# 51616/split-vae

Hardware: AMD Instinct MI355X
Metric: images/sec training step, SPLIT-VAE CelebA-64 bs512 (higher is better)
Workload: dtype f32 operands, f32 accumulate (exact-fp32 MFMA v_mfma_f32_16x16x4_f32): the reference's precision (vae/model.py:12); 1 GPU; SPLIT-VAE CelebA-64 64x64 beta=120 patch_size=8 latents=128+128 lr=1e-4, full train step (scramble+fwd+ELBO+bwd+Adam), per-GPU batch 512; global_batch=512, per_gpu_batch=512, parallelism=dp1, reconstructions=not stored (dead after the fused loss)

## Files before the change

### split_vae_amd/csrc/kernels.h

```cpp
#pragma once
#include <hip/hip_runtime.h>
#include <stdint.h>

#define SV_MAX_TAPS 81

struct TapGemmArgs {
  const void* A;
  const void* Wt;
  const float* bias;
  void* out;
  const void* mask;
  int M;
  int lOY, lOX;
  int OY, OX;
  int IH, IW, lda;
  int cl2;
  int P;
  int Ktot;
  int S, SX;
  int N;
  int OHF, OWF, OS, ooy, oox, ldo;
  int act, out_f32, splitk, ntaps;
  int ups;
  int d2s;
  int d2s_y;
  int clampin;
  int s2d3;
  const float* nll_img; void* nll_grad; float* nll_part; int nll_ch; float nll_gscale;
  int nll_noout;
  const float* fix;
  const float* fix2; int fix_nc, fix_pad;
  int cls_n;
  int accum;
  int adj;
  int8_t dy[SV_MAX_TAPS];
  int8_t dx[SV_MAX_TAPS];
};
int svk_tap_gemm(const TapGemmArgs& a, int dtype, int cfg, hipStream_t st);
#define SV_TAP_MAX_MULTI 4
struct TapGemmMulti {
  TapGemmArgs a[SV_TAP_MAX_MULTI];
  int zbase[SV_TAP_MAX_MULTI];
  int n;
};
int svk_tap_gemm_multi(const TapGemmArgs* a, int n, int dtype, int cfg, hipStream_t st);

struct TileConvArgs {
  const void* A; const void* Wt; const float* bias; void* out; const void* mask;
  int B, IH, IW, lda;
  int cl2, P, Ktot, S, SX;
  int lTW, lTH, lNB;
  int OY, OX, tilesX, tilesY, ntiles;
  int TIW, TIH, y_lo, x_lo;
  int PS;
  int plane_bytes;
  int nph, lnph;
  int xcd_chunk;
  int off_bytes, in_bytes;
  int buf_bytes;
  int wslots;
  int N, OHF, OWF, OS, ooy, oox, ldo, act, out_f32, ntaps;
  int dbg;
  int ups;
  int d2s;
  int cls_n;
  int d2s_y, clampin;
  int s2d3;
  int dma;
  const float* fix;
  const float* fix2; int fix_nc, fix_pad;
  const float* nll_img; void* nll_grad; float* nll_part; int nll_ch; float nll_gscale; int nll_noout;
  int8_t dy[SV_MAX_TAPS];
  int8_t dx[SV_MAX_TAPS];
};
#define SV_MAX_MULTI 8
#define SV_SHARED_STREAMS 3
hipStream_t sv_shared_stream(int k);
struct TileConvMulti { TileConvArgs a[SV_MAX_MULTI]; };
bool svk_tile_conv_plan(const TapGemmArgs& t, int dtype, int B, TileConvArgs* a, int* cfg_out);
int svk_tile_conv_multi(const TileConvArgs* a, int n, int dtype, int cfg, hipStream_t st);
int svk_conv_dispatch_multi(const TapGemmArgs* t, int n, int dtype, int tap_cfg, hipStream_t st);
int svk_tile_conv(const TileConvArgs& a, int dtype, int cfg, hipStream_t st);
int svk_row_conv_try(const TapGemmArgs* t, int n, int dtype, hipStream_t st);
bool svk_row_conv_supported(const TapGemmArgs* t, int n, int dtype);
int svk_conv_dispatch(const TapGemmArgs& t, int dtype, int tap_cfg, hipStream_t st);

struct WgradArgs {
  const void* A;
  const void* dY;
  float* dW;
  float* dbias;
  int M, lOY, lOX, OY, OX, IH, IW, lda, S, SX;
  int fold_kw, fold_c;
  int ldy, ycols;
  int cl2;
  int Cin_pad, Cin_real, N, Nrows;
  int ntaps, msplit;
  int ups;
  int clampin;
  int dy_s2d;
  int dy_os, dy_oy, dy_ox;
  int assign;
  int s2d3;
  float* ws;
  int64_t ws_bytes;
  hipEvent_t ev_mid[2];
  struct WgradReduceDesc* defer; int* n_defer;
  int8_t dy[SV_MAX_TAPS];
  int8_t dx[SV_MAX_TAPS];
};
int svk_wgrad(const WgradArgs& a, int dtype, int cfg, hipStream_t st);
#define SV_WGRAD_IM2COL_MAX_MULTI 4
struct WgradMulti {
  WgradArgs a[SV_WGRAD_IM2COL_MAX_MULTI];
  int zbase[SV_WGRAD_IM2COL_MAX_MULTI];
  int plain[SV_WGRAD_IM2COL_MAX_MULTI];
  int n;
};
int svk_wgrad_multi(const WgradArgs* a, int n, int dtype, int cfg, hipStream_t st);

struct WgradTileArgs {
  const void* A; const void* dY; float* dW; float* dbias;
  float* slab; float* ws; int64_t ws_bytes;
  float* bslab;
  struct WgradReduceDesc* defer; int* n_defer;
  int B, IH, IW, lda, cl2, S, SX, fold_kw, fold_c;
  int layer_id;
  int contig;
  int pairx;
  int lTW, lTH, lNB, OY, OX, tilesX, tilesY, ntiles;
  int TIW, TIH, y_lo, x_lo, PS;
  int ldy, YS, lycp;
  int in_bytes, dy_bytes;
  int dbg;
  int ups;
  int clampin, dy_s2d, assign;
  int dy_os, dy_oy, dy_ox;
  int s2d3;
// ... 131 lines not shown
```

### split_vae_amd/csrc/tile_conv.hip

```cpp
#include "common.hip.h"
#include "kernels.h"
#include "tile_stage.hip.h"
#include "dlogistic.hip.h"
#include <stdio.h>
#include <stdlib.h>
#include <string.h>

#ifndef SV_TC_PPS16
#define SV_TC_PPS16 16
#endif
#ifndef SV_TC_PPS32
#define SV_TC_PPS32 8
#endif
#ifndef SV_TC_PPS64
#define SV_TC_PPS64 8
#endif
#ifndef SV_TC_EPI_BATCH
#define SV_TC_EPI_BATCH 8
#endif
static __host__ __device__ constexpr int tile_pps(int BN, int YR = 0) {
  return YR ? (BN == 16 || YR == 5 ? YR * 4 : 8) : BN == 16 ? SV_TC_PPS16 : BN == 32 ? SV_TC_PPS32 : BN == 64 ? SV_TC_PPS64 : 8;
}

template <int PPS>
__device__ __forceinline__ int wpiece(int q, int n) {
  if constexpr (PPS % 8 == 0) return q ^ (n & 7);
  else return (q & ~7) == (PPS & ~7) ? (q & ~3) | ((q & 3) ^ (n & 3)) : q ^ (n & 7);
}

template <typename T> struct MmaOpT;
template <> struct MmaOpT<bf16_t> {
  static __device__ __forceinline__ void run(const uint4& a, const uint4& b, f32x4& c) {
    c = __builtin_amdgcn_mfma_f32_16x16x32_bf16(__builtin_bit_cast(bf16x8, a), __builtin_bit_cast(bf16x8, b), c, 0, 0, 0);
  }
};
template <> struct MmaOpT<float> {
  static __device__ __forceinline__ void run(const uint4& a, const uint4& b, f32x4& c) {
    const float4 af = __builtin_bit_cast(float4, a), bf = __builtin_bit_cast(float4, b);
    c = __builtin_amdgcn_mfma_f32_16x16x4f32(af.x, bf.x, c, 0, 0, 0);
    c = __builtin_amdgcn_mfma_f32_16x16x4f32(af.y, bf.y, c, 0, 0, 0);
    c = __builtin_amdgcn_mfma_f32_16x16x4f32(af.z, bf.z, c, 0, 0, 0);
    c = __builtin_amdgcn_mfma_f32_16x16x4f32(af.w, bf.w, c, 0, 0, 0);
  }
};

static constexpr int tile_min_waves(int BN, int NW, int YR, bool WR = false) { return (YR || WR) && NW == 4 ? (BN == 64 ? 3 : 4) : 1; }
template <typename T, int BN, int MF, int NW, int YR, bool WR, bool FX = false>
__global__ __launch_bounds__(64 * NW, tile_min_waves(BN, NW, YR, WR)) void tile_conv_kernel(const TileConvMulti mg) {
  const TileConvArgs& g = mg.a[blockIdx.z];
  if (SV_DBG(g.dbg) & 32) return;
  constexpr int NT = 64 * NW, WM = 16 * MF, BM = NW * WM, NF = BN / 16;
  constexpr int PPS = tile_pps(BN, YR), RB = PPS * 16;
  constexpr int RPP = NT / PPS;
  constexpr int BRN = (BN + RPP - 1) / RPP;
  constexpr int EPP = ElemTraits<T>::EPP;
  extern __shared__ __attribute__((aligned(16))) char smem[];
  char* sB = smem;
  int* sOff = (int*)(smem + g.wslots * BN * RB);
  char* sIn = smem + g.wslots * BN * RB + g.off_bytes;

  const int tid = threadIdx.x, lane = tid & 63, wave = tid >> 6;
  int t = blockIdx.x;
  if (g.xcd_chunk) {
    const int remapped = (t & 7) * g.xcd_chunk + (t >> 3);
    t = remapped < g.ntiles && (g.ntiles & 7) == 0 ? remapped : t;
  }
  const int tx0 = (t % g.tilesX) << g.lTW; t /= g.tilesX;
  const int ty0 = (t % g.tilesY) << g.lTH; t /= g.tilesY;
  const int b0 = t << g.lNB;
  const int n0 = blockIdx.y * BN;
  const int TW = 1 << g.lTW, TH = 1 << g.lTH, NB = 1 << g.lNB;
  const int cpp = 1 << g.cl2;

  const T* __restrict__ Wb = (const T*)g.Wt;
  const int nph = g.nph, lcH = g.cl2 - g.lnph;
  const int gP = g.P >> g.lnph, gKtot = g.Ktot, gdbg = SV_DBG(g.dbg);
  const int pp = tid % PPS, r0 = tid / PPS;
  int ph = 0;
  uint4 rbA[BRN];
  auto load_b = [&](int ks, uint4 (&rb)[BRN]) {
    const int pl = ks * PPS + pp;
    const bool pv = pl < gP;
    const int p = ((pl >> lcH) << g.cl2) + (ph << lcH) + (pl & ((1 << lcH) - 1));
#pragma unroll
    for (int i = 0; i < BRN; ++i) {
      const int n = r0 + RPP * i;
      rb[i] = (pv && n < BN && r0 < RPP) ? *(const uint4*)(Wb + (int64_t)(n0 + n) * gKtot + (int64_t)p * EPP) : make_uint4(0, 0, 0, 0);
    }
  };
  auto write_b = [&](int slot, const uint4 (&rb)[BRN]) {
#pragma unroll
    for (int i = 0; i < BRN; ++i) {
      const int n = r0 + RPP * i;
      if (n < BN && r0 < RPP) *(uint4*)(sB + slot * (BN * RB) + n * RB + (wpiece<PPS>(pp, n) << 4)) = rb[i];
    }
  };
  const int nk = (gdbg & 2) ? 0 : (gP + PPS - 1) / PPS;
  constexpr int WRMAX = 6;
  constexpr bool wres = WR && YR == 0;
  uint4 rbw[wres ? WRMAX - 1 : 1][BRN];
  load_b(0, rbA);
  if constexpr (wres) {
#pragma unroll
    for (int ks = 1; ks < WRMAX; ++ks) load_b(ks, rbw[ks - 1]);
  }

  const int nkp = (gP + PPS - 1) / PPS * PPS;
  for (int p = tid; p < nkp; p += NT) {
    int off = 0;
    if (p < gP) {
      const int tap = p >> lcH, c = p & ((1 << lcH) - 1);
      const int tp = ((int)g.dy[tap] - g.y_lo) * g.TIW + ((int)g.dx[tap] - g.x_lo);
      off = g.plane_bytes ? tp * 32 + (c >> 1) * g.plane_bytes + (c & 1) * 16 : tp * g.PS + c * 16;
    }
    sOff[p] = off;
  }
  auto stage = [&](int phase) {
    if (SV_DBG(g.dbg) & 1) return;
    const TileStageGeom sg = {g.B, g.IH, g.IW, g.lda, lcH, g.TIW, g.TIH, g.PS, NB, g.plane_bytes};
    const int iy_base = ty0 * g.S + g.y_lo, ix_base = tx0 * g.SX + g.x_lo;
    const T* Ap = (const T*)g.A + ((phase << lcH) * EPP);
    if constexpr (sizeof(T) == 4) {
      if (g.s2d3) { stage_tile_s2d3<NT>((const float*)g.A, sg, b0, iy_base, ix_base, sIn, tid); return; }
    }
    if (g.ups) stage_tile_upsampled<T, NT>(Ap, sg, b0, iy_base, ix_base, sIn, tid);
    else if (sizeof(T) == 4 && g.dma) {
      const int wv = __builtin_amdgcn_readfirstlane(wave);
      if (g.clampin) stage_tile_plain_dma<T, NW, true>(Ap, sg, b0, iy_base, ix_base, sIn, lane, wv);
      else stage_tile_plain_dma<T, NW, false>(Ap, sg, b0, iy_base, ix_base, sIn, lane, wv);
    }
    else if (g.clampin) stage_tile_plain<T, NT, true>(Ap, sg, b0, iy_base, ix_base, sIn, tid);
    else stage_tile_plain<T, NT>(Ap, sg, b0, iy_base, ix_base, sIn, tid);
  };
  stage(0);
  const int lr = lane & 15, lg = lane >> 4;
  int lbase[MF];
#pragma unroll
  for (int i = 0; i < MF; ++i) {
    const int r = wave * WM + i * 16 + lr;
    const int tx = r & (TW - 1), ty = (r >> g.lTW) & (TH - 1), bl = r >> (g.lTW + g.lTH);
    lbase[i] = ((bl * g.TIH + ty * g.S) * g.TIW + tx * g.SX) * g.PS;
  }

  f32x4 acc[MF][NF];
#pragma unroll
  for (int i = 0; i < MF; ++i)
#pragma unroll
    for (int j = 0; j < NF; ++j) acc[i][j] = (f32x4){0.f, 0.f, 0.f, 0.f};

  auto compute = [&](int ks, int slot) {
    const char* cB = sB + slot * (BN * RB);
#pragma unroll
    for (int kk = 0; kk < PPS / 4; ++kk) {
      const int off = sOff[ks * PPS + kk * 4 + lg];
      uint4 af[MF], bfr[NF];
#pragma unroll
      for (int i = 0; i < MF; ++i) af[i] = *(const uint4*)(sIn + lbase[i] + off);
#pragma unroll
      for (int j = 0; j < NF; ++j) {
        const int n = j * 16 + lr;
        bfr[j] = *(const uint4*)(cB + n * RB + (wpiece<PPS>(kk * 4 + lg, n) << 4));
      }
#pragma unroll
      for (int i = 0; i < MF; ++i)
#pragma unroll
        for (int j = 0; j < NF; ++j) MmaOpT<T>::run(bfr[j], af[i], acc[i][j]);
    }
  };
  constexpr int SPG = YR ? YR * 4 / PPS : 1, TPS = PPS / 4;
  const int rowpitch = g.TIW * g.PS;
  for (ph = 0; ph < nph; ++ph) {
    if (ph) {
      load_b(0, rbA);
      stage(ph);
    }
    write_b(0, rbA);
    if constexpr (wres) {
#pragma unroll
      for (int ks = 1; ks < WRMAX; ++ks)
        if (ks < nk) write_b(ks, rbw[ks - 1]);
    }
    __syncthreads();
    if constexpr (YR > 0) {
      for (int gq = 0; gq * SPG < nk; ++gq) {
        uint4 aw[MF + YR - 1];
        const char* wp = sIn + lbase[0] + sOff[gq * (YR * 4) + lg];
#pragma unroll
        for (int iy = 0; iy < MF + YR - 1; ++iy) aw[iy] = *(const uint4*)(wp + iy * rowpitch);
#pragma unroll
        for (int sg = 0; sg < SPG; ++sg) {
          const int ks = gq * SPG + sg;
          const bool more = ks + 1 < nk;
          if (more) load_b(ks + 1, rbA);
          const char* cB = sB + (ks & 1) * (BN * RB);
#pragma unroll
          for (int kk = 0; kk < TPS; ++kk) {
            uint4 bfr[NF];
#pragma unroll
            for (int j = 0; j < NF; ++j) {
              const int n = j * 16 + lr;
              bfr[j] = *(const uint4*)(cB + n * RB + (wpiece<PPS>(kk * 4 + lg, n) << 4));
            }
#pragma unroll
            for (int i = 0; i < MF; ++i)
#pragma unroll
              for (int j = 0; j < NF; ++j) MmaOpT<T>::run(bfr[j], aw[i + sg * TPS + kk], acc[i][j]);
          }
          if (more) write_b((ks & 1) ^ 1, rbA);
          __syncthreads();
        }
      }
    } else if constexpr (wres) {
      for (int ks = 0; ks < nk; ++ks) compute(ks, ks);
      __syncthreads();
    } else
    for (int ks = 0; ks < nk; ++ks) {
      const bool more = ks + 1 < nk && !(gdbg & 8);
      if (more) load_b(ks + 1, rbA);
      compute(ks, ks & 1);
      if (more) write_b((ks & 1) ^ 1, rbA);
      if (!(gdbg & 16)) __syncthreads();
    }
    if (nk == 0) __syncthreads();
  }
// ... 277 lines not shown
  return true;
}
static bool tile_conv_plan_impl(const TapGemmArgs& t, int dtype, int B, TileConvArgs* a, int* cfg_out, bool narrow, int64_t* lds_out) {
  if (t.splitk != 1 || t.accum) return false;
  if (t.lOY < 0 || t.lOX < 0 || t.S > 2) return false;
  const int OY = 1 << t.lOY, OX = 1 << t.lOX;
  if (t.ups && t.S != 1) return false;
  if (t.d2s && ((t.N != 16 && !(t.N == 32 && t.d2s_y)) || !t.out_f32)) return false;
  if (t.d2s_y && (!t.d2s || t.N != 32 || ((2 * t.d2s * 4) & 7))) return false;
  if (t.clampin && (t.ups || t.S != 1)) return false;
  if (t.s2d3 && (dtype != SV_F32 || t.S != 1 || t.SX != 1 || t.ups || t.clampin || t.cl2 != 2)) return false;
  if (t.fix_nc && !t.d2s_y && (dtype != SV_F32 || !t.fix || !t.fix2 || (t.N & 15) || t.out_f32)) return false;
  if (t.nll_part && (!t.d2s_y || t.d2s != 6 || OY * OX < 256 || !t.nll_img || !t.nll_grad)) return false;
  if (t.cls_n && (t.OS != 2 || t.N != 4 * t.cls_n || (t.cls_n & 7) || t.out_f32 || t.bias)) return false;
  if (OY * OX < 16) return false;
  if (!t.d2s && !t.cls_n) {
    const int oe = t.out_f32 ? 4 : (dtype == SV_BF16 ? 2 : 4);
    const int nst = (t.N & 7) ? (t.ldo < ((t.N + 7) & ~7) ? t.ldo : ((t.N + 7) & ~7)) : t.N;
    if ((nst * oe) & 7) return false;
  }
  const int esz = dtype == SV_BF16 ? 2 : 4, epp = 16 / esz;
  const int cin = (1 << t.cl2) * epp;
  int BN, cfgN;
  static const int small_wgs = SV_TUNE_INT("SV_TC_SMALL_WGS", 200);
  const int64_t wgs128 = (((int64_t)B * OY * OX + 127) / 128) * (t.N / 128);
  static const bool small_f32 = SV_TUNE_INT("SV_TC_SMALL_F32", 1) != 0;
  const bool small = t.N % 128 == 0 && (wgs128 < small_wgs || narrow) && (dtype == SV_BF16 || small_f32) && !t.cls_n;
  static const int tiny_wgs = SV_TUNE_INT("SV_TC_TINY_WGS", 100);
  const bool tiny = small && wgs128 < tiny_wgs;
  static const int small64_wgs = SV_TUNE_INT("SV_TC_SMALL64_WGS", 300);
  const int64_t wgs64 = (((int64_t)B * OY * OX + 127) / 128) * (t.N / 64);
  static const int small64_s = SV_TUNE_INT("SV_TC_SMALL64_S", 1);
  const bool tiny64 = dtype == SV_F32 && t.N % 64 == 0 && t.N % 128 != 0 && wgs64 < small64_wgs && !t.cls_n && !t.d2s && t.OS == 1 && (!small64_s || t.S == small64_s);
  if (t.N % 128 == 0 && !small) { BN = 128; cfgN = 0; }
  else if (t.N % 64 == 0 && !tiny && !tiny64) { BN = 64; cfgN = 1; }
  else if (t.N % 32 == 0) { BN = 32; cfgN = 2; }
  else if (t.N <= 16) { BN = 16; cfgN = 3; }
  else return false;
  int y_lo = 127, y_hi = -127, x_lo = 127, x_hi = -127;
  for (int i = 0; i < t.ntaps; ++i) {
    y_lo = t.dy[i] < y_lo ? t.dy[i] : y_lo; y_hi = t.dy[i] > y_hi ? t.dy[i] : y_hi;
    x_lo = t.dx[i] < x_lo ? t.dx[i] : x_lo; x_hi = t.dx[i] > x_hi ? t.dx[i] : x_hi;
  }
  static const bool s2pad = !SV_TUNE_FLAG("SV_TC_NO_S2PAD"), p64 = SV_TUNE_FLAG("SV_TC_PAD64");
  const int pb = cin * esz;
  static const bool planar_on = !SV_TUNE_FLAG("SV_TC_NO_PLANAR");
  auto layout = [&](int bytes, bool* planar_out) {
    const bool pl = planar_on && t.SX == 1 && t.S == 1 && bytes >= 64;
    *planar_out = pl;
    return pl ? 32 : bytes + (t.SX == 1 ? ((bytes >= 128 || (bytes == 64 && p64)) ? 32 : 0) : ((bytes % 32 == 0 && s2pad) ? 16 : 0));
  };
  const int lTW = OX >= 16 ? 4 : t.lOX;
  const int off_bytes = (((t.P + 31) / 32 * 32) * 4 + 15) / 16 * 16;
  static const char* mf2 = SV_TUNE_STR("SV_TC_MF2", nullptr);
  for (int MF = 4; MF >= 2; MF -= 2) {
    static const bool big128 = SV_TUNE_FLAG("SV_TC_BN128_MF4");
    if (MF == 4 && BN == 128 && !(big128 && dtype == SV_BF16)) continue;
    if (MF == 4 && mf2 && strchr(mf2, BN == 16 ? 'a' : BN == 32 ? 'b' : 'c')) continue;
    if (MF == 4 && small) continue;
    if (MF == 4 && BN == 32 && OY * OX <= 256 && t.OS == 2 && !t.d2s_y) continue;
    const int BM = 64 * MF;
    int lTH = 0;
    while ((1 << (lTW + lTH)) < BM && (1 << lTH) < OY) ++lTH;
    int lNB = 0;
    while ((1 << (lTW + lTH + lNB)) < BM) ++lNB;
    const int TW = 1 << lTW, TH = 1 << lTH, NB = 1 << lNB;
    if (t.nll_part && (BM != 256 || NB != 1)) return false;
    const int TIW = (TW - 1) * t.SX + (x_hi - x_lo) + 1, TIH = (TH - 1) * t.S + (y_hi - y_lo) + 1;
    int yr = 0;
    static const char* yr_off = SV_TUNE_STR("SV_TC_NO_YR", "a");
    if (dtype == SV_BF16 && MF == 4 && t.S == 1 && lTW == 4 && TH >= MF && cin >= 32 && BN <= 64 &&
        !(yr_off && (yr_off[0] == '1' || strchr(yr_off, BN == 16 ? 'a' : BN == 32 ? 'b' : 'c')))) {
      int kh = 1;
      while (kh < t.ntaps && t.dx[kh] == t.dx[0]) ++kh;
      bool ok = (kh == 4 || kh == 6) && t.ntaps % kh == 0;
      for (int i = 0; i < t.ntaps && ok; ++i)
        ok = t.dx[i] == t.dx[i / kh * kh] && t.dy[i] == t.dy[0] + i % kh && t.dy[0] == y_lo;
      if (ok) yr = kh;
    }
    static const int nph_max = SV_TUNE_INT("SV_TC_NPH", 4);
    const int64_t wgs = (int64_t)(OX / TW) * (OY / TH) * ((B + NB - 1) / NB) * ((t.N + BN - 1) / BN);
    static const int small32_wgs = SV_TUNE_INT("SV_TC_SMALL32_WGS", 300);
    if (MF == 4 && BN == 32 && dtype == SV_F32 && !t.nll_part && wgs < small32_wgs) continue;
    int lnph = 0, PS = 0, plane_bytes = 0;
    int64_t in_bytes = 0;
    bool planar = false;
    for (;; ++lnph) {
      if (yr) lnph = t.cl2 - 2;
      const int pbh = pb >> lnph;
      PS = layout(pbh, &planar);
      plane_bytes = planar ? NB * TIH * TIW * 32 : 0;
      in_bytes = planar ? (int64_t)plane_bytes * (pbh / 32) : (int64_t)NB * TIH * TIW * PS;
      static const int ph_kb = SV_TUNE_INT("SV_TC_PH_KB", 53);
      static const bool s2_phases = !SV_TUNE_FLAG("SV_TC_NPH_NO_S2");
      static const int ph_wgs = SV_TUNE_INT("SV_TC_PH_WGS", 256);
      const int64_t tot = in_bytes + 2 * BN * tile_pps(BN) * 16 + off_bytes;
      if (yr || t.s2d3 || !((2 << lnph) <= nph_max && (pbh >> 1) >= 32 && (planar || s2_phases) &&
                            ((wgs >= ph_wgs && tot > ph_kb * 1024) || tot > 150 * 1024))) break;
    }
    static const bool wres_on = !SV_TUNE_FLAG("SV_TC_NO_WRES");
    const int nks = (int)(((t.P >> lnph) + tile_pps(BN) - 1) / tile_pps(BN));
    const int wslots = (wres_on && !yr && dtype == SV_BF16 && BN == 32 && MF == 4 && t.S == 1 && lnph == 0 && nks > 2 && nks <= 6 && nks * BN * tile_pps(BN) * 16 <= 24 * 1024) ? nks : 2;
    const int64_t lds = (int64_t)wslots * BN * tile_pps(BN, yr) * 16 + off_bytes + in_bytes;
    if (lds > 78 * 1024 && MF == 4 && BN >= 64) continue;
    static const bool s2_mf4 = SV_TUNE_FLAG("SV_TC_S2_MF4");
    if (lds > 78 * 1024 && MF == 4 && t.S == 2 && t.fix_nc && !s2_mf4) continue;
    *lds_out = lds;
    if (lds > 150 * 1024) {
      if (MF == 4) continue;
      if (SV_TUNE_FLAG("SV_TC_VERBOSE")) fprintf(stderr, "tile_conv plan: REFUSED (LDS %lld) N=%d cin=%d S=%d ntaps=%d\n", (long long)lds, t.N, cin, t.S, t.ntaps);
      return false;
    }
    memset(a, 0, sizeof(*a));
    a->A = t.A; a->Wt = t.Wt; a->bias = t.bias; a->out = t.out; a->mask = t.mask;
    a->B = B; a->IH = t.IH; a->IW = t.IW; a->lda = t.lda;
    a->cl2 = t.cl2; a->P = t.P; a->Ktot = t.Ktot; a->S = t.S; a->SX = t.SX; a->d2s = t.d2s; a->cls_n = t.cls_n; a->d2s_y = t.d2s_y; a->clampin = t.clampin; a->fix = t.fix;
    a->fix2 = t.fix2; a->fix_nc = t.d2s_y ? 0 : t.fix_nc; a->fix_pad = t.fix_pad; a->s2d3 = t.s2d3;
    a->nll_img = t.nll_img; a->nll_grad = t.nll_grad; a->nll_part = t.nll_part; a->nll_ch = t.nll_ch; a->nll_gscale = t.nll_gscale; a->nll_noout = t.nll_noout;
    a->lTW = lTW; a->lTH = lTH; a->lNB = lNB;
    a->OY = OY; a->OX = OX;
    a->tilesX = OX / TW; a->tilesY = OY / TH;
    a->ntiles = a->tilesX * a->tilesY * ((B + NB - 1) / NB);
    a->TIW = TIW; a->TIH = TIH; a->y_lo = y_lo; a->x_lo = x_lo; a->PS = PS; a->plane_bytes = plane_bytes;
    a->nph = 1 << lnph; a->lnph = lnph; a->wslots = wslots;
    {
      static const bool no_dma = SV_TUNE_FLAG("SV_TC_NO_DMA");
      a->dma = (!no_dma && dtype == SV_F32 && !t.ups && !t.s2d3 && (planar || PS == (pb >> lnph))) ? 1 : 0;
    }
    if (SV_TUNE_FLAG("SV_TC_VERBOSE")) fprintf(stderr, "tile_conv plan: yr=%d wslots=%d N=%d BN=%d MF=%d cin=%d pb=%d planar=%d nph=%d tile=%dx%dx%d PS=%d in_bytes=%lld lds=%lld ntiles=%d S=%d SX=%d\n", yr, wslots, t.N, BN, MF, cin, pb, (int)planar, 1 << lnph, NB, TIH, TIW, PS, (long long)in_bytes, (long long)lds, a->ntiles, t.S, t.SX);
    {
      static const bool xcd = !SV_TUNE_FLAG("SV_TC_NO_XCD");
      a->xcd_chunk = (xcd && a->ntiles >= 64 && (a->ntiles & 7) == 0) ? a->ntiles / 8 : 0;
    }
    a->off_bytes = off_bytes; a->in_bytes = (int)in_bytes;
    a->N = t.N; a->OHF = t.OHF; a->OWF = t.OWF; a->OS = t.OS; a->ooy = t.ooy; a->oox = t.oox; a->ldo = t.ldo;
    a->act = t.act; a->out_f32 = t.out_f32; a->ntaps = t.ntaps; a->ups = t.ups;
    memcpy(a->dy, t.dy, sizeof(a->dy));
    memcpy(a->dx, t.dx, sizeof(a->dx));
    *cfg_out = cfgN * 2 + (MF == 4 ? 0 : 1) + (yr == 4 ? 32 : yr == 6 ? 64 : 0) + (wslots > 2 ? 128 : 0);
    static const char* nw8 = SV_TUNE_STR("SV_TC_NW8", nullptr);
    if (MF == 4 && dtype == SV_BF16 && nw8 && strchr(nw8, BN == 16 ? 'a' : BN == 32 ? 'b' : BN == 64 ? 'c' : 'd')) *cfg_out = 16 + cfgN;
    return true;
  }
  return false;
}

int svk_tile_conv_multi(const TileConvArgs* a, int n, int dtype, int cfg, hipStream_t st) {
  if (n < 1 || n > SV_MAX_MULTI) return SV_E_BADARG;
  if (dtype == SV_BF16) {
    switch (cfg) {
      case 0: return launch_tile<bf16_t, 128, 4>(a, n, st);
      case 1: return launch_tile<bf16_t, 128, 2>(a, n, st);
      case 2: return launch_tile<bf16_t, 64, 4>(a, n, st);
      case 3: return launch_tile<bf16_t, 64, 2>(a, n, st);
      case 4: return launch_tile<bf16_t, 32, 4>(a, n, st);
      case 5: return launch_tile<bf16_t, 32, 2>(a, n, st);
      case 7: return launch_tile<bf16_t, 16, 2>(a, n, st);
      case 6: return launch_tile<bf16_t, 16, 4>(a, n, st);
      case 128 + 4: return launch_tile<bf16_t, 32, 4, 4, 0, true>(a, n, st);
      case 32 + 2: return launch_tile<bf16_t, 64, 4, 4, 4>(a, n, st);
      case 32 + 4: return launch_tile<bf16_t, 32, 4, 4, 4>(a, n, st);
      case 32 + 6: return launch_tile<bf16_t, 16, 4, 4, 4>(a, n, st);
      case 64 + 2: return launch_tile<bf16_t, 64, 4, 4, 6>(a, n, st);
      case 64 + 4: return launch_tile<bf16_t, 32, 4, 4, 6>(a, n, st);
      case 64 + 6: return launch_tile<bf16_t, 16, 4, 4, 6>(a, n, st);
      case 16: return launch_tile<bf16_t, 128, 2, 8>(a, n, st);
      case 17: return launch_tile<bf16_t, 64, 2, 8>(a, n, st);
      case 18: return launch_tile<bf16_t, 32, 2, 8>(a, n, st);
      case 19: return launch_tile<bf16_t, 16, 2, 8>(a, n, st);
    }
  } else if (dtype == SV_F32) {
    switch (cfg) {
      case 1: return launch_tile<float, 128, 2>(a, n, st);
      case 2: return launch_tile<float, 64, 4>(a, n, st);
      case 3: return launch_tile<float, 64, 2>(a, n, st);
      case 4: return launch_tile<float, 32, 4>(a, n, st);
      case 5: return launch_tile<float, 32, 2>(a, n, st);
      case 7: return launch_tile<float, 16, 2>(a, n, st);
      case 6: return launch_tile<float, 16, 4>(a, n, st);
    }
  }
  return SV_E_BADARG;
}

int svk_tile_conv(const TileConvArgs& a, int dtype, int cfg, hipStream_t st) { return svk_tile_conv_multi(&a, 1, dtype, cfg, st); }

static const char* tile_form(const TapGemmArgs& t) { return t.s2d3 ? "tile_s2d3" : (t.d2s && !t.d2s_y) ? "tile_packx" : "tile"; }

int svk_conv_dispatch_multi(const TapGemmArgs* t, int n, int dtype, int tap_cfg, hipStream_t st) {
  const bool force_tap = sv_tune_force_im2col(), no_multi = sv_tune_no_multi();
  static const int dbg = SV_TUNE_INT("SV_TC_DBG", 0);
  if (n < 1 || n > SV_MAX_MULTI) return SV_E_BADARG;
  if (!force_tap && n <= 8) {
    const int rc = svk_row_conv_try(t, n, dtype, st);
    if (rc != SV_E_UNSUPPORTED) {
      sv_trace_note("row");
      return rc;
    }
  }
  for (int i = 0; i < n; ++i)
    if (t[i].adj) return SV_E_UNSUPPORTED;
  TileConvArgs a[SV_MAX_MULTI];
  int cfg[SV_MAX_MULTI];
  bool all_tile = !force_tap;
  for (int i = 0; i < n && all_tile; ++i) {
    all_tile = svk_tile_conv_plan(t[i], dtype, t[i].M / (t[i].OY * t[i].OX), &a[i], &cfg[i]);
    a[i].dbg = dbg;
    if (all_tile && i > 0 && (cfg[i] != cfg[0] || a[i].ntiles != a[0].ntiles || a[i].N != a[0].N)) all_tile = false;
  }
  if (all_tile && !no_multi) {
    sv_trace_note(tile_form(t[0]));
    return svk_tile_conv_multi(a, n, dtype, cfg[0], st);
// ... 38 lines not shown
```

### split_vae_amd/csrc/tile_stage.hip.h

```cpp
#pragma once
#include "common.hip.h"

struct TileStageGeom {
  int B, IH, IW, lda;
  int cl2;
  int TIW, TIH, PS;
  int NB;
  int plane_bytes;
};
__device__ __forceinline__ int tile_piece_off(const TileStageGeom& s, int pixel, int c) {
  return s.plane_bytes ? (c >> 1) * s.plane_bytes + pixel * 32 + (c & 1) * 16 : pixel * s.PS + c * 16;
}

template <typename T, int NT = 256, bool CLAMP = false>
__device__ __forceinline__ void stage_tile_plain(const T* __restrict__ Ab, const TileStageGeom& s, int b0, int iy_base,
                                                 int ix_base, char* sIn, int tid) {
  constexpr int EPP = ElemTraits<T>::EPP;
  const int cpp = 1 << s.cl2;
  const int ppr = s.TIW * cpp;
  const int LPR = ppr > 160 ? 64 : 32, lLPR = ppr > 160 ? 6 : 5;
  const int srow = tid >> lLPR, slane = tid & (LPR - 1), rows_pp = NT >> lLPR;
  const int nrows = s.NB * s.TIH;
  for (int row = srow; row < nrows; row += rows_pp) {
    int bl = 0, iyl = row;
    while (iyl >= s.TIH) { iyl -= s.TIH; ++bl; }
    const int iy = CLAMP ? min(max(iy_base + iyl, 0), s.IH - 1) : iy_base + iyl, b = b0 + bl;
    const bool rok = b < s.B && (unsigned)iy < (unsigned)s.IH;
    const T* src = Ab + ((int64_t)(b * s.IH + iy) * s.IW) * s.lda;
    const int prow = row * s.TIW;
    for (int pc0 = slane; pc0 < ppr; pc0 += LPR * 4) {
      uint4 v[4];
#pragma unroll
      for (int u = 0; u < 4; ++u) {
        const int pc = pc0 + u * LPR;
        const int ixl = pc >> s.cl2, c = pc & (cpp - 1), ix = CLAMP ? min(max(ix_base + ixl, 0), s.IW - 1) : ix_base + ixl;
        v[u] = make_uint4(0, 0, 0, 0);
        if (pc < ppr && rok && (unsigned)ix < (unsigned)s.IW) v[u] = *(const uint4*)(src + (int64_t)ix * s.lda + c * EPP);
      }
#pragma unroll
      for (int u = 0; u < 4; ++u) {
        const int pc = pc0 + u * LPR;
        if (pc < ppr) *(uint4*)(sIn + tile_piece_off(s, prow + (pc >> s.cl2), pc & (cpp - 1))) = v[u];
      }
    }
  }
}

__device__ __forceinline__ void stage_dma16(const void* gsrc, char* lds_wave_base) {
  __builtin_amdgcn_global_load_lds((const __attribute__((address_space(1))) void*)gsrc, (__attribute__((address_space(3))) void*)lds_wave_base, 16, 0, 0);
}
template <typename T, int NW = 4, bool CLAMP = false>
__device__ __forceinline__ void stage_tile_plain_dma(const T* __restrict__ Ab, const TileStageGeom& s, int b0, int iy_base, int ix_base, char* sIn, int lane, int wave) {
  constexpr int EPP = ElemTraits<T>::EPP;
  const float inv_h = 1.0f / (float)s.TIH;
  auto piece = [&](int row, int ixl, int c, char* lds_wave_base, char* lds_lane) {
    const int bl = (int)(((float)row + 0.5f) * inv_h), iyl = row - bl * s.TIH, b = b0 + bl;
    int iy = iy_base + iyl, ix = ix_base + ixl;
    bool ok = b < s.B;
    if (CLAMP) { iy = min(max(iy, 0), s.IH - 1); ix = min(max(ix, 0), s.IW - 1); }
    else ok = ok && (unsigned)iy < (unsigned)s.IH && (unsigned)ix < (unsigned)s.IW;
    if (ok) stage_dma16(Ab + ((int64_t)(b * s.IH + iy) * s.IW + ix) * s.lda + c * EPP, lds_wave_base);
    else *(uint4*)lds_lane = make_uint4(0, 0, 0, 0);
  };
  if (s.plane_bytes) {
    const int slots = s.NB * s.TIH * s.TIW * 2, ipp = (slots + 63) >> 6, nplanes = 1 << (s.cl2 - 1);
    const float inv_w = 1.0f / (float)s.TIW;
    int plane = 0, k = wave;
    while (k >= ipp) { k -= ipp; ++plane; }
    while (plane < nplanes) {
      const int slot = k * 64 + lane;
      if (slot < slots) {
        const int p = slot >> 1, row = (int)(((float)p + 0.5f) * inv_w);
        piece(row, p - row * s.TIW, plane * 2 + (slot & 1), sIn + plane * s.plane_bytes + k * 1024, sIn + plane * s.plane_bytes + slot * 16);
      }
      k += NW;
      while (k >= ipp) { k -= ipp; ++plane; }
    }
    return;
  }
  const int cpp = 1 << s.cl2, ppr = s.TIW << s.cl2, total = s.NB * s.TIH * ppr;
  const float inv_row = 1.0f / (float)ppr;
  for (int base = wave * 64; base < total; base += NW * 64) {
    const int L = base + lane;
    if (L >= total) continue;
    const int row = (int)(((float)L + 0.5f) * inv_row), r = L - row * ppr;
    piece(row, r >> s.cl2, r & (cpp - 1), sIn + base * 16, sIn + L * 16);
  }
}

template <int NT = 256>
__device__ __forceinline__ void stage_tile_s2d3(const float* __restrict__ Ab, const TileStageGeom& s, int b0, int iy_base, int ix_base, char* sIn, int tid) {
  const int total = s.NB * s.TIH * s.TIW * 4;
  const float inv_row = 1.0f / (float)(s.TIW * 4), inv_h = 1.0f / (float)s.TIH;
  constexpr int U = 4;
  for (int it0 = tid; it0 < total; it0 += NT * U) {
    float4 v[U];
    int pix[U], par[U];
#pragma unroll
    for (int u = 0; u < U; ++u) {
      const int it = it0 + u * NT;
      const int row = (int)(((float)it + 0.5f) * inv_row), r = it - row * (s.TIW * 4);
      const int bl = (int)(((float)row + 0.5f) * inv_h), iyl = row - bl * s.TIH;
      const int ixl = r >> 2, p = r & 3, iy = iy_base + iyl, ix = ix_base + ixl, b = b0 + bl;
      v[u] = make_float4(0.f, 0.f, 0.f, 0.f);
      if (it < total && b < s.B && (unsigned)iy < (unsigned)s.IH && (unsigned)ix < (unsigned)s.IW)
        v[u] = *(const float4*)(Ab + (((int64_t)b * (2 * s.IH) + 2 * iy + (p >> 1)) * (2 * s.IW) + 2 * ix + (p & 1)) * 8);
      pix[u] = it < total ? row * s.TIW + ixl : -1;
      par[u] = p;
    }
#pragma unroll
    for (int u = 0; u < U; ++u) {
      if (pix[u] < 0) continue;
      const float f[3] = {v[u].x, v[u].y, v[u].z};
#pragma unroll
      for (int c = 0; c < 3; ++c) {
        const int ch = par[u] * 3 + c;
        *(float*)(sIn + tile_piece_off(s, pix[u], ch >> 2) + (ch & 3) * 4) = f[c];
      }
      if (par[u] == 0) *(float4*)(sIn + tile_piece_off(s, pix[u], 3)) = make_float4(0.f, 0.f, 0.f, 0.f);
    }
  }
}

template <typename T>
__device__ __forceinline__ void blend2x2(const uint4& a00, const uint4& a01, const uint4& a10, const uint4& a11, uint4 (&out)[2][2]) {
  constexpr int NP = Piece<T>::NP;
  f32x2 v00[NP], v01[NP], v10[NP], v11[NP];
  Piece<T>::unpack(a00, v00); Piece<T>::unpack(a01, v01); Piece<T>::unpack(a10, v10); Piece<T>::unpack(a11, v11);
#pragma unroll
  for (int dxb = 0; dxb < 2; ++dxb) {
    const float fx = dxb ? 0.75f : 0.25f;
    f32x2 top[NP], bot[NP], r0[NP], r1[NP];
#pragma unroll
    for (int e = 0; e < NP; ++e) {
      top[e] = lerp2(v00[e], v01[e], fx);
      bot[e] = lerp2(v10[e], v11[e], fx);
      r0[e] = lerp2(top[e], bot[e], 0.25f);
      r1[e] = lerp2(top[e], bot[e], 0.75f);
    }
    out[0][dxb] = Piece<T>::pack(r0);
    out[1][dxb] = Piece<T>::pack(r1);
  }
}

template <typename T, int NT = 256>
__device__ __forceinline__ void stage_tile_upsampled_cols(const T* __restrict__ Ab, const TileStageGeom& s, int b0, int iy_base,
                                                          int ix_base, char* sIn, int tid) {
  constexpr int EPP = ElemTraits<T>::EPP, NP = Piece<T>::NP;
  const int cpp = 1 << s.cl2;
  const int LH = s.IH >> 1, LW = s.IW >> 1;
  const int i_lo = (iy_base - 1) >> 1, nbi = ((iy_base + s.TIH - 2) >> 1) - i_lo + 1;
  const int j_lo = (ix_base - 1) >> 1, nbj = ((ix_base + s.TIW - 2) >> 1) - j_lo + 1;
  const int ncols = s.NB * nbj * cpp;
  int nrg = NT / ncols;
  nrg = nrg < 1 ? 1 : nrg > nbi ? nbi : nrg;
  const int rpg = (nbi + nrg - 1) / nrg;
// ... 115 lines not shown
```

Measured before the change: 57610 images/s.

## Split staged input tile columns by parity for stride-2 fp32 convolutions

For stride-2 fp32 tile convolutions, the staged LDS input tile now stores even and odd columns in separate halves of each row. Adjacent output pixels then read contiguous LDS positions instead of positions two pixels apart, which is meant to cut LDS bank conflicts in the MFMA operand loads. The offset table, per-lane base addresses and both staging paths (plain and DMA) are updated for the remapped layout. It forces a planar 32-byte layout, can pad the tile by one column, and is gated off for large backward fix-up launches and some MF=4 configurations.

New measurement: 57640 images/s (median of 3 runs). Within noise of the previous version (+0.1%).

```diff
diff --git a/split_vae_amd/csrc/kernels.h b/split_vae_amd/csrc/kernels.h
--- a/split_vae_amd/csrc/kernels.h
+++ b/split_vae_amd/csrc/kernels.h
@@ -54,6 +54,7 @@
   int TIW, TIH, y_lo, x_lo;
   int PS;
   int plane_bytes;
+  int TIWh;
   int nph, lnph;
   int xcd_chunk;
   int off_bytes, in_bytes;
diff --git a/split_vae_amd/csrc/tile_conv.hip b/split_vae_amd/csrc/tile_conv.hip
--- a/split_vae_amd/csrc/tile_conv.hip
+++ b/split_vae_amd/csrc/tile_conv.hip
@@ -73,7 +73,7 @@
   const int cpp = 1 << g.cl2;
 
   const T* __restrict__ Wb = (const T*)g.Wt;
-  const int nph = g.nph, lcH = g.cl2 - g.lnph;
+  const int nph = g.nph, gcl2 = g.cl2, lcH = gcl2 - g.lnph;
   const int gP = g.P >> g.lnph, gKtot = g.Ktot, gdbg = SV_DBG(g.dbg);
   const int pp = tid % PPS, r0 = tid / PPS;
   int ph = 0;
@@ -81,7 +81,7 @@
   auto load_b = [&](int ks, uint4 (&rb)[BRN]) {
     const int pl = ks * PPS + pp;
     const bool pv = pl < gP;
-    const int p = ((pl >> lcH) << g.cl2) + (ph << lcH) + (pl & ((1 << lcH) - 1));
+    const int p = ((pl >> lcH) << gcl2) + (ph << lcH) + (pl & ((1 << lcH) - 1));
 #pragma unroll
     for (int i = 0; i < BRN; ++i) {
       const int n = r0 + RPP * i;
@@ -105,19 +105,21 @@
     for (int ks = 1; ks < WRMAX; ++ks) load_b(ks, rbw[ks - 1]);
   }
 
+  const int TIWh = sizeof(T) == 4 ? g.TIWh : 0, rowrec = TIWh ? 2 * TIWh : g.TIW;
   const int nkp = (gP + PPS - 1) / PPS * PPS;
   for (int p = tid; p < nkp; p += NT) {
     int off = 0;
     if (p < gP) {
       const int tap = p >> lcH, c = p & ((1 << lcH) - 1);
-      const int tp = ((int)g.dy[tap] - g.y_lo) * g.TIW + ((int)g.dx[tap] - g.x_lo);
+      const int dxo = (int)g.dx[tap] - g.x_lo;
+      const int tp = ((int)g.dy[tap] - g.y_lo) * rowrec + (TIWh ? (dxo & 1) * TIWh + (dxo >> 1) : dxo);
       off = g.plane_bytes ? tp * 32 + (c >> 1) * g.plane_bytes + (c & 1) * 16 : tp * g.PS + c * 16;
     }
     sOff[p] = off;
   }
   auto stage = [&](int phase) {
     if (SV_DBG(g.dbg) & 1) return;
-    const TileStageGeom sg = {g.B, g.IH, g.IW, g.lda, lcH, g.TIW, g.TIH, g.PS, NB, g.plane_bytes};
+    const TileStageGeom sg = {g.B, g.IH, g.IW, g.lda, lcH, g.TIW, g.TIH, g.PS, NB, g.plane_bytes, TIWh};
     const int iy_base = ty0 * g.S + g.y_lo, ix_base = tx0 * g.SX + g.x_lo;
     const T* Ap = (const T*)g.A + ((phase << lcH) * EPP);
     if constexpr (sizeof(T) == 4) {
@@ -139,7 +141,7 @@
   for (int i = 0; i < MF; ++i) {
     const int r = wave * WM + i * 16 + lr;
     const int tx = r & (TW - 1), ty = (r >> g.lTW) & (TH - 1), bl = r >> (g.lTW + g.lTH);
-    lbase[i] = ((bl * g.TIH + ty * g.S) * g.TIW + tx * g.SX) * g.PS;
+    lbase[i] = ((bl * g.TIH + ty * g.S) * rowrec + (TIWh ? tx : tx * g.SX)) * g.PS;
   }
 
   f32x4 acc[MF][NF];
@@ -583,14 +585,21 @@
     const int64_t wgs = (int64_t)(OX / TW) * (OY / TH) * ((B + NB - 1) / NB) * ((t.N + BN - 1) / BN);
     static const int small32_wgs = SV_TUNE_INT("SV_TC_SMALL32_WGS", 300);
     if (MF == 4 && BN == 32 && dtype == SV_F32 && !t.nll_part && wgs < small32_wgs) continue;
+    static const bool s2split_on = !SV_TUNE_FLAG("SV_TC_NO_S2SPLIT");
+    static const int s2split_bwd_wgs = SV_TUNE_INT("SV_TC_S2SPLIT_BWD_WGS", 1024);
+    const int TIWh = (TIW + 1) / 2, TIWp = 2 * TIWh;
+    const bool s2split = s2split_on && planar_on && dtype == SV_F32 && t.S == 2 && t.SX == 2 && !t.ups && !t.s2d3 && (lTW >= 3 || (lTW == 2 && (TIWp & 3))) &&
+                         !(t.fix_nc && (((int64_t)B * OY * OX + 127) / 128) * ((t.N + BN - 1) / BN) >= s2split_bwd_wgs);
     int lnph = 0, PS = 0, plane_bytes = 0;
     int64_t in_bytes = 0;
-    bool planar = false;
+    bool planar = false, split = false;
     for (;; ++lnph) {
       if (yr) lnph = t.cl2 - 2;
       const int pbh = pb >> lnph;
+      split = s2split && pbh >= 32;
       PS = layout(pbh, &planar);
-      plane_bytes = planar ? NB * TIH * TIW * 32 : 0;
+      if (split) { planar = true; PS = 32; }
+      plane_bytes = planar ? NB * TIH * (split ? TIWp : TIW) * 32 : 0;
       in_bytes = planar ? (int64_t)plane_bytes * (pbh / 32) : (int64_t)NB * TIH * TIW * PS;
       static const int ph_kb = SV_TUNE_INT("SV_TC_PH_KB", 53);
       static const bool s2_phases = !SV_TUNE_FLAG("SV_TC_NPH_NO_S2");
@@ -605,7 +614,7 @@
     const int64_t lds = (int64_t)wslots * BN * tile_pps(BN, yr) * 16 + off_bytes + in_bytes;
     if (lds > 78 * 1024 && MF == 4 && BN >= 64) continue;
     static const bool s2_mf4 = SV_TUNE_FLAG("SV_TC_S2_MF4");
-    if (lds > 78 * 1024 && MF == 4 && t.S == 2 && t.fix_nc && !s2_mf4) continue;
+    if ((lds > 78 * 1024 || split) && MF == 4 && t.S == 2 && t.fix_nc && !s2_mf4) continue;
     *lds_out = lds;
     if (lds > 150 * 1024) {
       if (MF == 4) continue;
@@ -622,13 +631,13 @@
     a->OY = OY; a->OX = OX;
     a->tilesX = OX / TW; a->tilesY = OY / TH;
     a->ntiles = a->tilesX * a->tilesY * ((B + NB - 1) / NB);
-    a->TIW = TIW; a->TIH = TIH; a->y_lo = y_lo; a->x_lo = x_lo; a->PS = PS; a->plane_bytes = plane_bytes;
+    a->TIW = TIW; a->TIH = TIH; a->y_lo = y_lo; a->x_lo = x_lo; a->PS = PS; a->plane_bytes = plane_bytes; a->TIWh = split ? TIWh : 0;
     a->nph = 1 << lnph; a->lnph = lnph; a->wslots = wslots;
     {
       static const bool no_dma = SV_TUNE_FLAG("SV_TC_NO_DMA");
       a->dma = (!no_dma && dtype == SV_F32 && !t.ups && !t.s2d3 && (planar || PS == (pb >> lnph))) ? 1 : 0;
     }
-    if (SV_TUNE_FLAG("SV_TC_VERBOSE")) fprintf(stderr, "tile_conv plan: yr=%d wslots=%d N=%d BN=%d MF=%d cin=%d pb=%d planar=%d nph=%d tile=%dx%dx%d PS=%d in_bytes=%lld lds=%lld ntiles=%d S=%d SX=%d\n", yr, wslots, t.N, BN, MF, cin, pb, (int)planar, 1 << lnph, NB, TIH, TIW, PS, (long long)in_bytes, (long long)lds, a->ntiles, t.S, t.SX);
+    if (SV_TUNE_FLAG("SV_TC_VERBOSE")) fprintf(stderr, "tile_conv plan: yr=%d wslots=%d N=%d BN=%d MF=%d cin=%d pb=%d planar=%d nph=%d tile=%dx%dx%d PS=%d in_bytes=%lld lds=%lld ntiles=%d S=%d SX=%d split=%d dma=%d\n", yr, wslots, t.N, BN, MF, cin, pb, (int)planar, 1 << lnph, NB, TIH, TIW, PS, (long long)in_bytes, (long long)lds, a->ntiles, t.S, t.SX, a->TIWh ? 2 * a->TIWh : 0, a->dma);
     {
       static const bool xcd = !SV_TUNE_FLAG("SV_TC_NO_XCD");
       a->xcd_chunk = (xcd && a->ntiles >= 64 && (a->ntiles & 7) == 0) ? a->ntiles / 8 : 0;
diff --git a/split_vae_amd/csrc/tile_stage.hip.h b/split_vae_amd/csrc/tile_stage.hip.h
--- a/split_vae_amd/csrc/tile_stage.hip.h
+++ b/split_vae_amd/csrc/tile_stage.hip.h
@@ -7,7 +7,11 @@
   int TIW, TIH, PS;
   int NB;
   int plane_bytes;
+  int TIWh;
 };
+__device__ __forceinline__ int tile_pixel(const TileStageGeom& s, int row, int col) {
+  return s.TIWh ? row * (2 * s.TIWh) + (col & 1) * s.TIWh + (col >> 1) : row * s.TIW + col;
+}
 __device__ __forceinline__ int tile_piece_off(const TileStageGeom& s, int pixel, int c) {
   return s.plane_bytes ? (c >> 1) * s.plane_bytes + pixel * 32 + (c & 1) * 16 : pixel * s.PS + c * 16;
 }
@@ -27,7 +31,6 @@
     const int iy = CLAMP ? min(max(iy_base + iyl, 0), s.IH - 1) : iy_base + iyl, b = b0 + bl;
     const bool rok = b < s.B && (unsigned)iy < (unsigned)s.IH;
     const T* src = Ab + ((int64_t)(b * s.IH + iy) * s.IW) * s.lda;
-    const int prow = row * s.TIW;
     for (int pc0 = slane; pc0 < ppr; pc0 += LPR * 4) {
       uint4 v[4];
 #pragma unroll
@@ -40,7 +43,7 @@
 #pragma unroll
       for (int u = 0; u < 4; ++u) {
         const int pc = pc0 + u * LPR;
-        if (pc < ppr) *(uint4*)(sIn + tile_piece_off(s, prow + (pc >> s.cl2), pc & (cpp - 1))) = v[u];
+        if (pc < ppr) *(uint4*)(sIn + tile_piece_off(s, tile_pixel(s, row, pc >> s.cl2), pc & (cpp - 1))) = v[u];
       }
     }
   }
@@ -63,15 +66,17 @@
     else *(uint4*)lds_lane = make_uint4(0, 0, 0, 0);
   };
   if (s.plane_bytes) {
-    const int slots = s.NB * s.TIH * s.TIW * 2, ipp = (slots + 63) >> 6, nplanes = 1 << (s.cl2 - 1);
-    const float inv_w = 1.0f / (float)s.TIW;
+    const int rw = s.TIWh ? 2 * s.TIWh : s.TIW;
+    const int slots = s.NB * s.TIH * rw * 2, ipp = (slots + 63) >> 6, nplanes = 1 << (s.cl2 - 1);
+    const float inv_w = 1.0f / (float)rw;
     int plane = 0, k = wave;
     while (k >= ipp) { k -= ipp; ++plane; }
     while (plane < nplanes) {
       const int slot = k * 64 + lane;
       if (slot < slots) {
-        const int p = slot >> 1, row = (int)(((float)p + 0.5f) * inv_w);
-        piece(row, p - row * s.TIW, plane * 2 + (slot & 1), sIn + plane * s.plane_bytes + k * 1024, sIn + plane * s.plane_bytes + slot * 16);
+        const int p = slot >> 1, row = (int)(((float)p + 0.5f) * inv_w), pos = p - row * rw;
+        const int col = !s.TIWh ? pos : pos < s.TIWh ? 2 * pos : 2 * (pos - s.TIWh) + 1;
+        if (col < s.TIW) piece(row, col, plane * 2 + (slot & 1), sIn + plane * s.plane_bytes + k * 1024, sIn + plane * s.plane_bytes + slot * 16);
       }
       k += NW;
       while (k >= ipp) { k -= ipp; ++plane; }
```
